# zhanwenchen/pbe

Hardware: AMD Instinct MI355X
Metric: 512x512 images/sec @50 PLMS steps scale=5 (higher is better)
Workload: dtype fp16; 1 GPU; BASELINE configs[1]: batch=4/GPU, 512x512, 50 PLMS steps (51 U-Net calls at batch 8), scale=5, fp16 activations + fp32 accumulate, name-seeded random-init U-Net + VAE + CLIP ViT-L/14 weights; the context-independent prefix of each guidance pair (first ResBlock + first self-attention) is evaluated once; per_gpu_batch=4, global_batch=4, plms_steps=50, parallelism=batch-sharded x1, no per-step collective

## Files before the change

### pbe_amd/csrc/attention.hip

```cpp
#include "common.h"
#include "../../include/pbe_hip.h"

struct AttnP {
    const h16* Q; const h16* K; const h16* VT; h16* O;
    int B, H, Nq, Nk, D;
    long q_bs, q_rs, k_bs, k_rs, vt_bs, vt_rs, o_bs, o_rs;
    float scale_log2e;
    int q_pre;
    int nqb;
#ifdef PBE_ATTN_STAMPS
    unsigned long long* stamps;
#endif
};

#define PBE_GLDS16(gsrc, ldst)                                                                     \
    __builtin_amdgcn_global_load_lds((const __attribute__((address_space(1))) void*)(gsrc),         \
                                     (__attribute__((address_space(3))) void*)(ldst), 16, 0, 0)

template <int DP>
struct AttnTile {
    static constexpr int KT = 64;
    static constexpr int DV = (DP + 31) / 32 * 32;
    static constexpr int DC = DP / 8;
    static constexpr int KR = DC | 1;
// ... 13 lines not shown
#endif

template <int DP, int QW, int KH, bool MPAD = false>
__global__ void __launch_bounds__(256, (QW == 2 && DP <= 48) ? 2 : 1) attn_kernel(const AttnP p) {
    using T = AttnTile<DP>;
    constexpr int KT = T::KT, DV = T::DV, KR = T::KR, VR = T::VR, KSTR = T::KSTR, VSTR = T::VSTR;
    constexpr int KSLOTS = T::KSLOTS, SLOTS = T::SLOTS, NPW = T::NPW, BUF = T::BUF;
    constexpr int K_BYTES = KSLOTS * 16;
    constexpr int NDS = DP / 16;
    constexpr int NDT = DV / 32;
    constexpr int BQ = 128 * QW;
    constexpr int NSLOT = 2 * KH;
    extern __shared__ __attribute__((aligned(16))) unsigned char smem[];

    const int tid = threadIdx.x, lane = tid & 63, wave = tid >> 6;
    const int l31 = lane & 31, h5 = lane >> 5;
    int bh, qblk;
    {
        const int nq = p.nqb, nbh = p.B * p.H, lin = blockIdx.x;
        if ((nbh & 7) == 0) { const int xcd = lin & 7, j = lin >> 3; qblk = j % nq; bh = (j / nq) * 8 + xcd; }
        else { qblk = lin % nq; bh = lin / nq; }
    }
    const int b = bh / p.H, h = bh - b * p.H;
    const int q0 = qblk * BQ + wave * 32 * QW + l31;
    const int D = p.D;
    const h16x8 zero8 = {0, 0, 0, 0, 0, 0, 0, 0};
    const h16x8 one8 = {1, 1, 1, 1, 1, 1, 1, 1};
    constexpr bool ONES = DV > DP;

    const h16* Qb = p.Q + (long)b * p.q_bs + (long)h * D;
    const h16* Kb = p.K + (long)b * p.k_bs + (long)h * D;
    const h16* Vb = p.VT + (long)b * p.vt_bs + (long)h * D * p.vt_rs;

    for (int i = tid; i < NSLOT * BUF / 16; i += 256) *reinterpret_cast<h16x8*>(smem + i * 16) = zero8;
    __syncthreads();
    if (ONES && tid < 8 * NSLOT)
        *reinterpret_cast<h16x8*>(smem + (tid >> 3) * BUF + K_BYTES + (DV - 1) * VSTR + (tid & 7) * 16) = one8;
    if constexpr (MPAD) {
        const h16x8 kpad = {(h16)64.f, 0, 0, 0, 0, 0, 0, 0};
        for (int i = tid; i < NSLOT * KT; i += 256)
            *reinterpret_cast<h16x8*>(smem + (i / KT) * BUF + (i % KT) * KSTR + (T::DC - 1) * 16) = kpad;
    }

    const h16* src[NPW];
    int inc[NPW];
#pragma unroll
    for (int j = 0; j < NPW; ++j) {
        const int slot = (j * 4 + wave) * 64 + lane;
        src[j] = nullptr; inc[j] = 0;
        if (slot < KSLOTS) {
            const int row = slot / KR, c = slot - row * KR;
            if (c * 8 < D) { src[j] = Kb + (long)attn_key_of_row(row) * p.k_rs + c * 8; inc[j] = KT * (int)p.k_rs; }
        } else if (slot < SLOTS) {
            const int sv = slot - KSLOTS, row = sv / VR, c = sv - row * VR;
            if (c < KT / 8 && row < D) { src[j] = Vb + (long)row * p.vt_rs + c * 8; inc[j] = KT; }
        }
    }
    const int nt = (p.Nk + KT - 1) / KT;
    const int rem = p.Nk - (nt - 1) * KT;
    auto issue_tile = [&](int t, int buf) {
        unsigned char* dst = smem + buf * BUF + wave * 1024;
        if (t + 1 < nt || rem == KT) {
#pragma unroll
            for (int j = 0; j < NPW; ++j) {
                if (src[j]) PBE_GLDS16(src[j], dst + j * 4096);
                src[j] += inc[j];
            }
        } else {
            const int kv0 = t * KT;
#pragma unroll
            for (int j = 0; j < NPW; ++j) {
                const int slot = (j * 4 + wave) * 64 + lane;
                const h16* s = nullptr;
                if (slot < KSLOTS) {
                    const int row = slot / KR, c = slot - row * KR;
                    const int key = min(kv0 + attn_key_of_row(row), p.Nk - 1);
                    if (c * 8 < D) s = Kb + (long)key * p.k_rs + c * 8;
                } else if (slot < SLOTS) {
                    const int sv = slot - KSLOTS, row = sv / VR, c = sv - row * VR;
                    if (c < KT / 8 && row < D && kv0 + c * 8 < p.Nk) s = Vb + (long)row * p.vt_rs + kv0 + c * 8;
                }
                if (s) PBE_GLDS16(s, dst + j * 4096);
            }
        }
    };
    auto fix_tail = [&](int buf) {
        unsigned char* sv = smem + buf * BUF + K_BYTES;
        for (int i = tid; i < DV * KT; i += 256) {
            const int row = i >> 6, col = i & 63;
            if (col >= rem) *reinterpret_cast<h16*>(sv + row * VSTR + col * 2) = (h16)0.f;
        }
    };

    h16x8 qf[QW][NDS];
#pragma unroll
    for (int i = 0; i < QW; ++i)
#pragma unroll
        for (int ds = 0; ds < NDS; ++ds) {
            const int d0 = ds * 16 + 8 * h5;
            const bool ok = (q0 + 32 * i) < p.Nq && d0 < D;
            const h16* qsrc = ok ? Qb + (long)(q0 + 32 * i) * p.q_rs + d0 : p.Q;
            h16x8 v = *reinterpret_cast<const h16x8*>(qsrc);
            v = ok ? v : zero8;
            if constexpr (MPAD) {
                if (!p.q_pre) {
#pragma unroll
                    for (int e = 0; e < 8; ++e) v[e] = (h16)((float)v[e] * p.scale_log2e);
                }
            }
            qf[i][ds] = v;
        }

    f32x16 o[QW][NDT];
    float m_run[QW], l_run[QW];
#pragma unroll
    for (int i = 0; i < QW; ++i) {
        m_run[i] = MPAD ? 0.f : -INFINITY; l_run[i] = 0.f;
#pragma unroll
        for (int dt = 0; dt < NDT; ++dt)
#pragma unroll
            for (int r = 0; r < 16; ++r) o[i][dt][r] = 0.f;
    }

    __syncthreads();
#pragma unroll
    for (int j = 0; j < KH; ++j)
        if (j < nt) issue_tile(j, j);
    __syncthreads();
    if (nt <= KH && rem < KT) { fix_tail(nt - 1); __syncthreads(); }

    constexpr bool PREF = DP <= 64, PREFV = DP <= 80;
    f32x16 sc[2];
    h16x8 pf[4];
    h16x8 kf[PREF ? 2 : 1][PREF ? NDS : 1];
    h16x8 vf[PREFV ? NDT : 1][4];
    auto load_k = [&](const unsigned char* sk) {
        if constexpr (PREF) {
#pragma unroll
            for (int ds = 0; ds < NDS; ++ds) {
                kf[0][ds] = *reinterpret_cast<const h16x8*>(sk + l31 * KSTR + (ds * 2 + h5) * 16);
                kf[1][ds] = *reinterpret_cast<const h16x8*>(sk + (32 + l31) * KSTR + (ds * 2 + h5) * 16);
            }
        }
    };
    auto load_v = [&](const unsigned char* sv) {
        if constexpr (PREFV) {
#pragma unroll
            for (int dt = 0; dt < NDT; ++dt)
#pragma unroll
                for (int ks = 0; ks < 4; ++ks)
                    vf[dt][ks] = *reinterpret_cast<const h16x8*>(sv + (dt * 32 + l31) * VSTR + h5 * 16 + ks * 32);
        }
    };
    auto qk = [&](int i, const unsigned char* sk) {
        f32x16& s0 = sc[0];
        f32x16& s1 = sc[1];
#pragma unroll
        for (int r = 0; r < 16; ++r) { s0[r] = 0.f; s1[r] = 0.f; }
        if constexpr (PREF) {
#pragma unroll
// ... 264 lines not shown
```

### pbe_amd/csrc/igemm.hip

```cpp
#include "igemm_kernel.h"

#ifdef PBE_STAMPS
unsigned long long* g_pbe_stamps = nullptr;
extern "C" int pbe_debug_set_stamps(void* buf) { g_pbe_stamps = (unsigned long long*)buf; return PBE_OK; }
#endif
int g_pbe_force_cfg = -1;
int g_pbe_allow_splitk = 1;
int g_pbe_pingpong = 1;
int g_pbe_mfast = 1;

extern "C" int pbe_tune(int32_t key, int32_t value) {
    if (key == 1) { g_pbe_force_cfg = (value >= 0 && (value & 255) < kNCfg) ? value : -1; return PBE_OK; }
    if (key == 2) { g_pbe_allow_splitk = value ? 1 : 0; return PBE_OK; }
    if (key == 3) { extern int g_pbe_attn_qw; g_pbe_attn_qw = value; return PBE_OK; }
    if (key == 4) { g_pbe_pingpong = value ? 1 : 0; return PBE_OK; }
    if (key == 5) { g_pbe_mfast = value ? 1 : 0; return PBE_OK; }
    if (key == 8) { extern int g_pbe_attn_pad_lds; g_pbe_attn_pad_lds = value > 0 ? value : 0; return PBE_OK; }
    if (key == 7) { extern int g_pbe_gn_rows; g_pbe_gn_rows = value >= 1 ? value : 16; return PBE_OK; }
    if (key == 10) { extern int g_pbe_gn_apply2_rows; g_pbe_gn_apply2_rows = value >= 0 ? value : 8; return PBE_OK; }
    if (key == 9) { extern int g_pbe_gn_apply_rows; g_pbe_gn_apply_rows = value >= 1 ? value : 4; return PBE_OK; }
    if (key == 6) { extern int g_pbe_attn_mpad; g_pbe_attn_mpad = value ? 1 : 0; return PBE_OK; }
    return pbe_set_error(PBE_EINVAL, "pbe_tune: unknown key %d", key);
}

static int fill_gemm(const pbe_gemm_desc* d, IGemmP& p, const char* who) {
    PBE_REQUIRE(d && d->A && d->W && d->C, "%s: null operand", who);
    PBE_REQUIRE(d->M > 0 && d->N > 0 && d->K > 0 && d->batch >= 1 && d->batch <= 65535, "%s: bad dims M=%d N=%d K=%d batch=%d", who, d->M, d->N, d->K, d->batch);
    PBE_REQUIRE(d->K % 8 == 0, "%s: K=%d must be a multiple of 8", who, d->K);
    PBE_REQUIRE(d->lda % 8 == 0 && d->ldw % 8 == 0 && al16(d->A) && al16(d->W), "%s: A/W must be 16-byte aligned with ld %% 8 == 0", who);
    PBE_REQUIRE(d->strideA % 8 == 0 && d->strideW % 8 == 0, "%s: batch strides of A/W must be multiples of 8", who);
    const int K1 = d->A2 ? d->K1 : d->K;
    if (d->A2) {
        PBE_REQUIRE(K1 > 0 && K1 < d->K && K1 % 32 == 0 && d->lda2 % 8 == 0 && al16(d->A2) && d->batch == 1,
                    "%s: split-K source needs K1 %% 32 == 0 (K1=%d), aligned A2, batch 1", who, K1);
    }
    PBE_REQUIRE(d->lda >= (d->A2 ? K1 : d->K) && d->ldw >= d->K, "%s: leading dims too small", who);
    PBE_REQUIRE(!d->rowvec || d->group_rows > 0, "%s: rowvec needs group_rows > 0", who);
    const bool geglu = d->act == PBE_ACT_GEGLU;
    const int Nout = geglu ? d->N / 2 : d->N;
    PBE_REQUIRE(!geglu || (d->N % 16 == 0 && !d->resid && !d->rowvec && !d->bias_per_row), "%s: GEGLU epilogue needs N %% 16 == 0 and no resid/rowvec", who);
    memset(&p, 0, sizeof(p));
    p.A = (const h16*)d->A; p.A2 = (const h16*)d->A2; p.W = (const h16*)d->W; p.C = (h16*)d->C;
    p.bias = d->bias; p.rowvec = (const h16*)d->rowvec; p.resid = (const h16*)d->resid;
    p.M = d->M; p.N = d->N; p.K = d->K; p.K1 = K1;
    p.lda = d->lda; p.lda2 = d->lda2; p.ldw = d->ldw; p.ldc = d->ldc; p.ldr = d->ldr;
    p.ldv = d->ldv; p.group_rows = d->group_rows > 0 ? d->group_rows : 1;
    p.sA = d->strideA; p.sW = d->strideW; p.sC = d->strideC; p.sR = d->strideR;
    p.alpha = d->alpha; p.act = d->act; p.bias_row = d->bias_per_row;
    PBE_REQUIRE(d->ldc >= (d->VT ? d->vt_col0 : Nout), "%s: ldc too small", who);
    p.vec = (Nout % 8 == 0) && (d->ldc % 8 == 0) && al16(d->C) && (d->strideC % 8 == 0) &&
            (!d->resid || ((d->ldr % 8 == 0) && al16(d->resid) && (d->strideR % 8 == 0)));
    p.ws = (float*)d->workspace;
    p.alpha_cols = d->alpha_cols;
// ... 229 lines not shown
```

### pbe_amd/csrc/igemm_kernel.h

```cpp
#pragma once
#include <type_traits>
#include <utility>
#include "common.h"
#include "../../include/pbe_hip.h"

struct IGemmP {
    const h16* A; const h16* A2; const h16* W; h16* C;
    const float* bias; const h16* rowvec; const h16* resid;
    int M, N, K, K1;
    long lda, lda2, ldw, ldc, ldr;
    int ldv, group_rows;
    long sA, sW, sC, sR;
    float alpha; int act; int bias_row; int vec;
    int H, Wd, C1, C2, Ho, Wo, cstride, pad, ups, cb;
    int phase;
    int th;
    const float* sa; const float* sw; long ssa, ssw;
    int splits; float* ws;
    int alpha_cols;
    const float* ln_stat;
    int ln_parts; long ln_ld;
    const float* ln_c1; float ln_eps; double ln_inv_k;
    long rstat_ld;
    float* rstat;
// ... 199 lines not shown
    constexpr int PA = BM / 8, PW = BN / 8;
    constexpr int LA = PA / NW, LW = (PW + NW - 1) / NW, LPT = LA + LW;
    constexpr int CLD = BN + 8;
    constexpr int RING = MODE == 2 ? 2 * HPA * 128 + S * W_BYTES : S * STAGE;
    static_assert(S >= 2 && S <= 4 && PA % NW == 0 && BM % 16 == 0 && BN % 16 == 0, "A pieces must divide over the waves (weight pieces may be padded)");
    static_assert(MODE != 2 || (HPA % 8 == 0 && HPA >= BM), "halo image must hold the tile");
    static_assert(EXF == 0 || (MODE == 0 && !F8), "extended epilogue: dense fp16 tiles only");
    static_assert(!EXM || (MODE == 0 && !EXS && (F8 || EXF == (EX_LN | EX_VT))), "MX-fp8 copy-out: the fp8 tiles and the q|k|v^T form");
    extern __shared__ __attribute__((aligned(16))) unsigned char smem[];

    const int tid = threadIdx.x, lane = tid & 63;
    const int wave = __builtin_amdgcn_readfirstlane(tid >> 6);
    const int wm = wave % NWM, wn = wave / NWM;
    PBE_ACC_DECL;
#if PBE_PRIO_MODE == 2
    if (NW == 8 && __builtin_amdgcn_readfirstlane(wave) >= 4) __builtin_amdgcn_s_setprio(1);
#endif
    PBE_STAMP(0);
    PBE_STAMP(7);
    int tile;
    {
        const int nwg = gridDim.x, id = blockIdx.x, q = nwg >> 3, r = nwg & 7, xcd = id & 7;
        tile = (xcd < r ? xcd * (q + 1) : r * (q + 1) + (xcd - r) * q) + (id >> 3);
    }
    const int tiles_m = gridDim.x / tiles_n;
    const int tn_i = p.m_fast ? tile / tiles_m : tile % tiles_n, tm_i = p.m_fast ? tile - tn_i * tiles_m : tile / tiles_n;
    const int m0 = tm_i * BM, n0 = tn_i * BN;
    const long bz = blockIdx.y;

    const int lrow = lane >> 3;
    const int gch = (lane & 7) ^ lrow;
    const h16* zsrc = reinterpret_cast<const h16*>(g_pbe_zero16);

    const h16* a_cur[LA];
    const h16* a_alt[LA];
#pragma unroll
    for (int i = 0; i < LA; ++i) {
        const int m = min(m0 + (wave * LA + i) * 8 + lrow, p.M - 1);
        a_cur[i] = p.A + bz * p.sA + (long)m * p.lda + gch * 8;
        a_alt[i] = p.A2 ? p.A2 + (long)m * p.lda2 + gch * 8 - p.K1 : a_cur[i];
    }
    int* tab = reinterpret_cast<int*>(smem + RING);
    float* svec = reinterpret_cast<float*>(smem + (RING > WM * CLD * 2 ? RING : WM * CLD * 2) + (MODE == 1 ? 9 * BM * 4 : 0));
    const int sv_ns = (p.rowvec && p.group_rows < BM) ? BM / p.group_rows : 1;
    if (MODE == 1) {
        const int hw = p.Ho * p.Wo, Hv = p.H << p.ups, Wv = p.Wd << p.ups;
        const int py = p.phase ? (int)(blockIdx.y >> 1) : 0, px = p.phase ? (int)(blockIdx.y & 1) : 0;
        for (int row = tid; row < BM; row += NT) {
            const int m = m0 + row;
            const bool rok = m < p.M;
            const int b = m / hw, rem = m - b * hw;
            const int oy = rem / p.Wo, ox = rem - oy * p.Wo;
            const int iy0 = oy * p.cstride - p.pad, ix0 = ox * p.cstride - p.pad;
            if (p.phase) {
#pragma unroll
                for (int tp = 0; tp < 4; ++tp) {
                    const int iy = oy - 1 + py + (tp >> 1), ix = ox - 1 + px + (tp & 1);
                    const bool ok = rok && (unsigned)iy < (unsigned)p.H && (unsigned)ix < (unsigned)p.Wd;
                    tab[tp * BM + row] = ok ? (b * p.H + iy) * p.Wd + ix : -1;
                }
                continue;
            }
#pragma unroll
            for (int tp = 0; tp < 9; ++tp) {
                const int iy = iy0 + tp / 3, ix = ix0 + tp % 3;
                const bool ok = rok && (unsigned)iy < (unsigned)Hv && (unsigned)ix < (unsigned)Wv;
                tab[tp * BM + row] = ok ? (b * p.H + (iy >> p.ups)) * p.Wd + (ix >> p.ups) : -1;
            }
        }
        __syncthreads();
    }
    const h16* w_row[LW];
#pragma unroll
    for (int i = 0; i < LW; ++i) {
        const int n = min(n0 + min(wave + NW * i, PW - 1) * 8 + lrow, p.N - 1);
        w_row[i] = p.W + bz * p.sW + (long)n * p.ldw + gch * 8;
    }
    const int nk_all = (p.K + 63) >> 6;
    int kt0 = 0, nk = nk_all;
    if (p.splits > 1) {
        const int per = (nk_all + p.splits - 1) / p.splits;
        kt0 = blockIdx.z * per;
        nk = min(nk_all, kt0 + per);
    }
    const int KB = MODE == 1 ? p.cb >> 6 : 1;
    const int ntap = (MODE == 1 && p.phase) ? 4 : 9;
    int tap = 0, c0 = 0, kj = 0;
    if (MODE == 1 && kt0 > 0) {
        const int per_blk = ntap * KB, cblk = kt0 / per_blk, r = kt0 - cblk * per_blk;
        tap = r / KB; kj = r - tap * KB; c0 = cblk * p.cb + kj * 64;
    }
    const h16* a_src[LA];
    int a_inc[LA];
    bool fresh = true;
#pragma unroll
    for (int i = 0; i < LA; ++i) { a_src[i] = zsrc; a_inc[i] = 0; }
    const bool ktail = (p.K & 63) != 0, straddle = p.A2 && (p.K1 & 63);
    const int kt_sw = p.A2 ? p.K1 >> 6 : 0x7fffffff;
    if (MODE == 0 && kt0 > kt_sw) {
#pragma unroll
        for (int i = 0; i < LA; ++i) a_cur[i] = a_alt[i];
    }

    auto issue = [&](int kt, int slot) {
        unsigned char* sa = smem + slot * STAGE;
        unsigned char* sw = sa + A_BYTES;
        const long k = (long)kt * 64;
        const bool slow = (ktail && kt == nk_all - 1) || (straddle && kt == kt_sw);
        const int kl = kt * 64 + gch * 8;
        if (MODE == 0) {
            if (kt == kt_sw && !straddle) {
#pragma unroll
                for (int i = 0; i < LA; ++i) a_cur[i] = a_alt[i];
            }
            if (!slow) {
#pragma unroll
                for (int i = 0; i < LA; ++i) PBE_GLDS16(a_cur[i] + k, sa + (wave * LA + i) * 1024);
            } else {
#pragma unroll
                for (int i = 0; i < LA; ++i) {
                    const h16* src = (kl < p.K1 ? a_cur[i] : a_alt[i]) + k;
                    PBE_GLDS16(kl < p.K ? src : zsrc, sa + (wave * LA + i) * 1024);
                }
                if (straddle && kt == kt_sw) {
#pragma unroll
                    for (int i = 0; i < LA; ++i) a_cur[i] = a_alt[i];
                }
            }
        } else {
            if (kj == 0 || fresh) {
                fresh = false;
                const bool first = c0 < p.C1;
                const h16* base = first ? p.A + c0 + gch * 8 : p.A2 + (c0 - p.C1) + gch * 8;
                const long cs = first ? p.C1 : p.C2;
#pragma unroll
                for (int i = 0; i < LA; ++i) {
                    const int pix = tab[tap * BM + (wave * LA + i) * 8 + lrow];
                    a_src[i] = pix >= 0 ? base + (long)pix * cs : zsrc;
                    a_inc[i] = pix >= 0 ? 64 : 0;
                }
            }
#pragma unroll
            for (int i = 0; i < LA; ++i) {
                PBE_GLDS16(a_src[i], sa + (wave * LA + i) * 1024);
                a_src[i] += a_inc[i];
            }
            c0 += 64;
            if (++kj == KB) {
                kj = 0;
                if (++tap == ntap) tap = 0; else c0 -= p.cb;
            }
        }
        if (!slow) {
#pragma unroll
            for (int i = 0; i < LW; ++i) PBE_GLDS16(w_row[i] + k, sw + min(wave + NW * i, PW - 1) * 1024);
        } else {
#pragma unroll
            for (int i = 0; i < LW; ++i) PBE_GLDS16(kl < p.K ? w_row[i] + k : zsrc, sw + min(wave + NW * i, PW - 1) * 1024);
        }
    };

    f32x4 acc[TN][TM];
#pragma unroll
    for (int i = 0; i < TN; ++i)
#pragma unroll
        for (int j = 0; j < TM; ++j) acc[i][j] = (f32x4){0.f, 0.f, 0.f, 0.f};

    const int fr = lane & 15, fq = lane >> 4;
    const int rsw = (fq ^ (fr & 7)) << 4;
    const int a_rd = (wm * WM + fr) * 128, w_rd = (wn * WN + fr) * 128;

    float* sca = svec + 4 * BN;
    float* scw = sca + BM;
    float* lnc = scw + BM;
    auto stage_svec = [&]() {
        if constexpr (F8) {
            for (int idx = tid; idx < BM + BN; idx += NT) {
                float v = 1.f;
                if (idx < BM) { if (p.sa && m0 + idx < p.M) v = p.sa[bz * p.ssa + m0 + idx]; sca[idx] = v; }
                else { const int c = idx - BM; if (p.sw && n0 + c < p.N) v = p.sw[bz * p.ssw + n0 + c]; scw[c] = v; }
            }
        }
        if constexpr (EXL) {
            if (p.ln_stat) {
                for (int idx = tid; idx < BM + BN; idx += NT) {
                    if (idx < BM) {
                        const int m = min(m0 + idx, p.M - 1);
                        float a = 0.f, q = 0.f;
                        for (int z = 0; z < p.ln_parts; ++z) {
                            const float2 t = *reinterpret_cast<const float2*>(p.ln_stat + 2 * ((long)z * p.ln_ld + m));
                            a += t.x; q += t.y;
                        }
                        const double mean = (double)a * p.ln_inv_k;
// ... 280 lines not shown
                            fa[ks][j] = *reinterpret_cast<const h16x8*>(ab + arow[j] * 128 + (((ks * 4 + fq) ^ (arow[j] & 7)) << 4));
#pragma unroll
                        for (int i = 0; i < TN; ++i) fw[ks][i] = *reinterpret_cast<const h16x8*>(sw + w_rd + (rsw ^ (ks * 64)) + i * 16 * 128);
                    }
                    __builtin_amdgcn_sched_barrier(0);
                    if (kt + D < nk2) issue_w(kt + D, slot_wr);
                    if (tap == 0 && next_a) issue_a(blk + 1, (blk + 1 - blk0) & 1);
                    __builtin_amdgcn_sched_barrier(0);
                    PBE_SETPRIO(1);
#pragma unroll
                    for (int i = 0; i < TN; ++i)
#pragma unroll
                        for (int j = 0; j < TM; ++j)
                            acc[i][j] = __builtin_amdgcn_mfma_f32_16x16x32_f16(fw[0][i], fa[0][j], acc[i][j], 0, 0, 0);
                    if constexpr (!BOTH) {
#pragma unroll
                        for (int j = 0; j < TM; ++j)
                            fa[0][j] = *reinterpret_cast<const h16x8*>(ab + arow[j] * 128 + (((4 + fq) ^ (arow[j] & 7)) << 4));
#pragma unroll
                        for (int i = 0; i < TN; ++i) fw[0][i] = *reinterpret_cast<const h16x8*>(sw + w_rd + (rsw ^ 64) + i * 16 * 128);
                    }
#pragma unroll
                    for (int i = 0; i < TN; ++i)
#pragma unroll
                        for (int j = 0; j < TM; ++j)
                            acc[i][j] = __builtin_amdgcn_mfma_f32_16x16x32_f16(fw[BOTH ? 1 : 0][i], fa[BOTH ? 1 : 0][j], acc[i][j], 0, 0, 0);
                    PBE_SETPRIO(0);
                    slot_rd = slot_rd + 1 == S ? 0 : slot_rd + 1;
                    slot_wr = slot_wr + 1 == S ? 0 : slot_wr + 1;
                }
            }
        }
    } else {
    PBE_STAMP(1);
#pragma unroll
    for (int t = 0; t < D; ++t)
        if (kt0 + t < nk) issue(kt0 + t, t);
    PBE_STAMP(2);
    stage_svec();
    int slot_rd = 0, slot_wr = D % S;
    for (int kt = kt0; kt < nk; ++kt) {
#ifdef PBE_STAMPS
        if (kt == kt0 + 1) PBE_STAMP(3);
#endif
        const int rem = min(nk - 1 - kt, D - 1);
        PBE_ACC_T0();
        if (D >= 3 && rem >= 2) wait_vmcnt<2 * LPT>();
        else if (D >= 2 && rem >= 1) wait_vmcnt<LPT>();
        else wait_vmcnt<0>();
        PBE_ACC(acc_w_);
        asm volatile("s_waitcnt lgkmcnt(0)" ::: "memory");
        PBE_ACC_T0();
        __builtin_amdgcn_s_barrier();
        PBE_ACC(acc_b2_);
        PBE_ACC_T0();
        const unsigned char* sa = smem + slot_rd * STAGE;
        const unsigned char* sw = sa + A_BYTES;
        h16x8 fa[BOTH ? 2 : 1][TM], fw[BOTH ? 2 : 1][TN];
#pragma unroll
        for (int ks = 0; ks < (BOTH ? 2 : 1); ++ks) {
#pragma unroll
            for (int j = 0; j < TM; ++j) fa[ks][j] = *reinterpret_cast<const h16x8*>(sa + a_rd + (rsw ^ (ks * 64)) + j * 16 * 128);
#pragma unroll
            for (int i = 0; i < TN; ++i) fw[ks][i] = *reinterpret_cast<const h16x8*>(sw + w_rd + (rsw ^ (ks * 64)) + i * 16 * 128);
        }
        __builtin_amdgcn_sched_barrier(0);
        if (kt + D < nk) issue(kt + D, slot_wr);
        __builtin_amdgcn_sched_barrier(0);
        PBE_ACC(acc_r_);
// ... 667 lines not shown
```

### pbe_amd/csrc/norm.hip

```cpp
#include "common.h"
#include "../../include/pbe_hip.h"

#define GN_MAX_C 4096
#define GN_MAX_CHUNKS 256

__device__ __forceinline__ const h16* gn_src(const h16* X, const h16* X2, int C1, int C2, long row, int v) {
    const int c = v * 8;
    return (c < C1) ? X + row * C1 + c : X2 + row * C2 + (c - C1);
}

__global__ void __launch_bounds__(256) gn_stats_kernel(const h16* X, const h16* X2, float* part, int HW, int C1, int C2,
                                                        int groups, int rows_per_block, int TX, int TY) {
    __shared__ float s_sum[GN_MAX_C], s_sq[GN_MAX_C];
    __shared__ float s_pa[256 * 8], s_pq[256 * 8];
    const int C = C1 + C2, C8 = C >> 3, cg = C / groups;
    const int tid = threadIdx.x, tx = tid % TX, ty = tid / TX;
    const int b = blockIdx.y, chunk = blockIdx.x;
    const int r0 = chunk * rows_per_block;
    const int r1 = min(HW, r0 + rows_per_block);
    if (ty < TY) {
        for (int v = tx; v < C8; v += TX) {
            float a[8], q[8];
#pragma unroll
            for (int e = 0; e < 8; ++e) { a[e] = 0.f; q[e] = 0.f; }
// ... 9 lines not shown
            }
            for (; r < r1; r += TY) {
                const h16x8 x = *reinterpret_cast<const h16x8*>(gn_src(X, X2, C1, C2, (long)b * HW + r, v));
#pragma unroll
                for (int e = 0; e < 8; ++e) { const float f = (float)x[e]; a[e] += f; q[e] += f * f; }
            }
            if (TY == 1) {
#pragma unroll
                for (int e = 0; e < 8; ++e) { s_sum[v * 8 + e] = a[e]; s_sq[v * 8 + e] = q[e]; }
            } else {
#pragma unroll
                for (int e = 0; e < 8; ++e) { s_pa[tid * 8 + e] = a[e]; s_pq[tid * 8 + e] = q[e]; }
            }
        }
    }
    __syncthreads();
    if (TY > 1) {
        for (int c = tid; c < C; c += 256) {
            const int v = c >> 3, e = c & 7;
            float a = 0.f, q = 0.f;
            for (int y = 0; y < TY; ++y) { a += s_pa[(y * TX + v) * 8 + e]; q += s_pq[(y * TX + v) * 8 + e]; }
            s_sum[c] = a; s_sq[c] = q;
        }
        __syncthreads();
    }
    if (tid < groups) {
        float a = 0.f, q = 0.f;
        for (int c = tid * cg; c < (tid + 1) * cg; ++c) { a += s_sum[c]; q += s_sq[c]; }
        float* dst = part + (((long)b * gridDim.x + chunk) * groups + tid) * 2;
        dst[0] = a; dst[1] = q;
    }
}

__global__ void __launch_bounds__(256) gn_apply_kernel(const h16* X, const h16* X2, const float* part, const float* gamma,
                                                        const float* beta, h16* Y, int HW, int C1, int C2, int groups,
                                                        int nchunks, int rows_per_block, int TX, int TY, float eps, int silu) {
    __shared__ float s_mean[64], s_rstd[64];
    __shared__ double s_a[256], s_q[256];
    const int C = C1 + C2, C8 = C >> 3, cg = C / groups;
    const int tid = threadIdx.x, tx = tid % TX, ty = tid / TX;
    const int b = blockIdx.y;
    {
        const int slices = 256 / groups;
        const int g = tid % groups, sl = tid / groups;
        double a = 0.0, q = 0.0;
        if (sl < slices)
            for (int c = sl; c < nchunks; c += slices) {
                const float* src = part + (((long)b * nchunks + c) * groups + g) * 2;
                a += (double)src[0]; q += (double)src[1];
            }
        s_a[tid] = a; s_q[tid] = q;
        __syncthreads();
        if (tid < groups) {
            double ta = 0.0, tq = 0.0;
            for (int s = 0; s < slices; ++s) { ta += s_a[s * groups + tid]; tq += s_q[s * groups + tid]; }
            const double n = (double)HW * cg;
            const double mean = ta / n;
            double var = tq / n - mean * mean;
            if (var < 0.0) var = 0.0;
            s_mean[tid] = (float)mean;
            s_rstd[tid] = (float)(1.0 / sqrt(var + (double)eps));
        }
        __syncthreads();
    }
    const int r0 = blockIdx.x * rows_per_block;
    const int r1 = min(HW, r0 + rows_per_block);
    if (ty >= TY) return;
    for (int v = tx; v < C8; v += TX) {
        float sc[8], sh[8];
#pragma unroll
        for (int e = 0; e < 8; ++e) {
            const int c = v * 8 + e, g = c / cg;
            const float a = s_rstd[g] * gamma[c];
            sc[e] = a; sh[e] = beta[c] - s_mean[g] * a;
        }
        int r = r0 + ty;
        for (; r + 3 * TY < r1; r += 4 * TY) {
            h16x8 x[4];
#pragma unroll
            for (int u = 0; u < 4; ++u) x[u] = *reinterpret_cast<const h16x8*>(gn_src(X, X2, C1, C2, (long)b * HW + r + u * TY, v));
#pragma unroll
            for (int u = 0; u < 4; ++u) {
                h16x8 y;
#pragma unroll
                for (int e = 0; e < 8; ++e) {
                    float f = (float)x[u][e] * sc[e] + sh[e];
                    if (silu) f = silu_f(f);
                    y[e] = (h16)f;
                }
                *reinterpret_cast<h16x8*>(Y + ((long)b * HW + r + u * TY) * C + v * 8) = y;
            }
        }
        for (; r < r1; r += TY) {
            const long row = (long)b * HW + r;
            const h16x8 x = *reinterpret_cast<const h16x8*>(gn_src(X, X2, C1, C2, row, v));
            h16x8 y;
#pragma unroll
            for (int e = 0; e < 8; ++e) {
                float f = (float)x[e] * sc[e] + sh[e];
                if (silu) f = silu_f(f);
                y[e] = (h16)f;
            }
            *reinterpret_cast<h16x8*>(Y + row * C + v * 8) = y;
        }
    }
}

#define GN_SMALL_ROWS 12
__global__ void __launch_bounds__(256) gn_small_kernel(const h16* X, const h16* X2, const float* gamma, const float* beta, h16* Y,
                                                        int HW, int C1, int C2, int groups, float eps, int silu) {
    __shared__ float s_a[4], s_q[4];
    const int C = C1 + C2, cg = C / groups, TX = cg >> 3, TY = 256 / TX;
    const int tid = threadIdx.x, lane = tid & 63, wave = tid >> 6;
    const int tx = tid % TX, ty = tid / TX;
    const int g = blockIdx.x, b = blockIdx.y;
    const int v = (g * cg >> 3) + tx;
    const bool act = ty < TY;
    h16x8 x[GN_SMALL_ROWS];
    float a = 0.f, q = 0.f;
#pragma unroll
    for (int u = 0; u < GN_SMALL_ROWS; ++u) {
        const int r = ty + u * TY;
        if (act && r < HW) {
            x[u] = *reinterpret_cast<const h16x8*>(gn_src(X, X2, C1, C2, (long)b * HW + r, v));
#pragma unroll
            for (int e = 0; e < 8; ++e) { const float f = (float)x[u][e]; a += f; q += f * f; }
        }
    }
    a = wave_sum(a); q = wave_sum(q);
    if (lane == 0) { s_a[wave] = a; s_q[wave] = q; }
    __syncthreads();
    const double n = (double)HW * cg;
    const double mean = ((double)s_a[0] + s_a[1] + s_a[2] + s_a[3]) / n;
    double var = ((double)s_q[0] + s_q[1] + s_q[2] + s_q[3]) / n - mean * mean;
    if (var < 0.0) var = 0.0;
    const float mu = (float)mean, rstd = (float)(1.0 / sqrt(var + (double)eps));
    if (!act) return;
    float sc[8], sh[8];
#pragma unroll
    for (int e = 0; e < 8; ++e) {
        const int c = v * 8 + e;
        sc[e] = rstd * gamma[c];
        sh[e] = beta[c] - mu * sc[e];
    }
#pragma unroll
    for (int u = 0; u < GN_SMALL_ROWS; ++u) {
        const int r = ty + u * TY;
        if (r < HW) {
            h16x8 y;
#pragma unroll
            for (int e = 0; e < 8; ++e) {
                float f = (float)x[u][e] * sc[e] + sh[e];
                if (silu) f = silu_f(f);
                y[e] = (h16)f;
            }
            *reinterpret_cast<h16x8*>(Y + ((long)b * HW + r) * C + v * 8) = y;
        }
    }
}

int g_pbe_gn_rows = 16;
int g_pbe_gn_apply2_rows = 8;
int g_pbe_gn_apply_rows = 4;
static void gn_geometry(int HW, int C, int* nchunks, int* rpb, int* TX, int* TY, int rows_per_thread = 0) {
    const int C8 = C / 8;
    *TX = C8 < 256 ? C8 : 256;
    *TY = 256 / *TX;
    int rows = *TY * (rows_per_thread > 0 ? rows_per_thread : g_pbe_gn_rows);
    if (rows < 32) rows = 32;
    int n = (HW + rows - 1) / rows;
    if (n > GN_MAX_CHUNKS) { n = GN_MAX_CHUNKS; rows = (HW + n - 1) / n; n = (HW + rows - 1) / rows; }
    *nchunks = n; *rpb = rows;
}

extern "C" size_t pbe_groupnorm_workspace_bytes(int32_t B, int32_t HW) {
    (void)HW;
    return (size_t)B * GN_MAX_CHUNKS * 64 * 2 * sizeof(float);
}

extern "C" int pbe_groupnorm_f16(const void* X, const void* X2, const float* gamma, const float* beta, void* Y, int32_t B,
                                 int32_t HW, int32_t C1, int32_t C2, int32_t groups, float eps, int32_t silu, void* workspace,
                                 size_t workspace_bytes, pbe_stream_t stream) {
    const int C = C1 + C2;
    PBE_REQUIRE(X && gamma && beta && Y && workspace, "pbe_groupnorm_f16: null operand");
    PBE_REQUIRE(B > 0 && HW > 0 && C1 > 0 && C2 >= 0, "pbe_groupnorm_f16: bad dims");
    PBE_REQUIRE((C2 == 0) == (X2 == nullptr), "pbe_groupnorm_f16: X2 / C2 mismatch");
    PBE_REQUIRE(C1 % 8 == 0 && C2 % 8 == 0 && C <= GN_MAX_C, "pbe_groupnorm_f16: C1=%d C2=%d must be multiples of 8, total <= %d", C1, C2, GN_MAX_C);
    PBE_REQUIRE(groups > 0 && groups <= 64 && C % groups == 0, "pbe_groupnorm_f16: groups=%d must divide C=%d (<= 64)", groups, C);
    PBE_REQUIRE(B <= 65535, "pbe_groupnorm_f16: batch too large");
    PBE_REQUIRE(workspace_bytes >= pbe_groupnorm_workspace_bytes(B, HW), "pbe_groupnorm_f16: workspace too small");
    hipStream_t s = (hipStream_t)stream;
    const int cg = C / groups;
    if (cg % 8 == 0 && cg / 8 <= 64 && HW <= GN_SMALL_ROWS * (256 / (cg / 8))) {
        pbe_prof_begin(PBE_K_GNORM, s);
        hipLaunchKernelGGL(gn_small_kernel, dim3(groups, B), dim3(256), 0, s, (const h16*)X, (const h16*)X2, gamma, beta, (h16*)Y, HW, C1, C2,
                           groups, eps, silu);
        pbe_prof_end(PBE_K_GNORM, s, 4.0 * B * (double)HW * C);
        PBE_LAUNCH_CHECK("pbe_groupnorm_f16");
        return PBE_OK;
    }
    int nchunks, rpb, TX, TY;
    gn_geometry(HW, C, &nchunks, &rpb, &TX, &TY);
    pbe_prof_begin(PBE_K_GNORM, s);
    hipLaunchKernelGGL(gn_stats_kernel, dim3(nchunks, B), dim3(256), 0, s, (const h16*)X, (const h16*)X2, (float*)workspace, HW, C1, C2,
                       groups, rpb, TX, TY);
    {
        int ac = nchunks, arpb = rpb, aTX = TX, aTY = TY;
        if (g_pbe_gn_apply2_rows > 0) gn_geometry(HW, C, &ac, &arpb, &aTX, &aTY, g_pbe_gn_apply2_rows);
        hipLaunchKernelGGL(gn_apply_kernel, dim3(ac, B), dim3(256), 0, s, (const h16*)X, (const h16*)X2, (const float*)workspace, gamma,
                           beta, (h16*)Y, HW, C1, C2, groups, nchunks, arpb, aTX, aTY, eps, silu);
    }
    pbe_prof_end(PBE_K_GNORM, s, 6.0 * B * (double)HW * C);
    PBE_LAUNCH_CHECK("pbe_groupnorm_f16");
    return PBE_OK;
}

extern "C" int pbe_groupnorm_apply_f16(const void* X, const float* partials, int32_t blocks, const float* gamma, const float* beta, void* Y,
                                       int32_t B, int32_t HW, int32_t C, int32_t groups, float eps, int32_t silu, pbe_stream_t stream) {
    PBE_REQUIRE(X && partials && gamma && beta && Y, "pbe_groupnorm_apply_f16: null operand");
    PBE_REQUIRE(B > 0 && B <= 65535 && HW > 0 && C > 0 && C % 8 == 0 && C <= GN_MAX_C && blocks > 0, "pbe_groupnorm_apply_f16: bad dims");
    PBE_REQUIRE(groups > 0 && groups <= 64 && C % groups == 0, "pbe_groupnorm_apply_f16: groups=%d must divide C=%d (<= 64)", groups, C);
    hipStream_t s = (hipStream_t)stream;
    int nchunks, rpb, TX, TY;
    gn_geometry(HW, C, &nchunks, &rpb, &TX, &TY, g_pbe_gn_apply_rows);
    pbe_prof_begin(PBE_K_GNORM, s);
    hipLaunchKernelGGL(gn_apply_kernel, dim3(nchunks, B), dim3(256), 0, s, (const h16*)X, (const h16*)nullptr, partials, gamma, beta, (h16*)Y, HW, C, 0,
                       groups, blocks, rpb, TX, TY, eps, silu);
    pbe_prof_end(PBE_K_GNORM, s, 4.0 * B * (double)HW * C);
    PBE_LAUNCH_CHECK("pbe_groupnorm_apply_f16");
    return PBE_OK;
}

template <int VPL>
__global__ void __launch_bounds__(256) layernorm_kernel(const h16* X, const float* gamma, const float* beta, h16* Y, long rows, int C,
                                                         long ldx, long ldy, float eps) {
    const int lane = threadIdx.x & 63;
    const long row = (long)blockIdx.x * 4 + (threadIdx.x >> 6);
    if (row >= rows) return;
    const int C8 = C >> 3;
    h16x8 x[VPL];
    float sum = 0.f;
#pragma unroll
    for (int i = 0; i < VPL; ++i) {
        const int v = lane + 64 * i;
        if (v < C8) {
            x[i] = *reinterpret_cast<const h16x8*>(X + row * ldx + v * 8);
#pragma unroll
            for (int e = 0; e < 8; ++e) sum += (float)x[i][e];
        }
    }
    const float mean = wave_sum(sum) / (float)C;
    float sq = 0.f;
#pragma unroll
    for (int i = 0; i < VPL; ++i) {
        const int v = lane + 64 * i;
        if (v < C8) {
#pragma unroll
// ... 207 lines not shown
```

Baseline: 7.923 images/sec.

## Hoist global loads ahead of LDS init in attention, igemm, and groupnorm kernels

In attention, Q fragments and the first K/V tile loads are issued before the shared-memory padding initialisation, which now writes only the pad regions. In igemm, the first weight tile load is issued before the A-address table build. Groupnorm apply and small kernels prefetch X rows and load gamma/beta as vectors before the statistics reduction, with a 4-way unrolled partial-sum read. The goal is to hide global-load latency behind setup work. Default apply rows and minimum rows change, launch bounds are added, and gamma/beta must now be 16-byte aligned, which adds register pressure and a new alignment requirement.

```diff
diff --git a/pbe_amd/csrc/attention.hip b/pbe_amd/csrc/attention.hip
--- a/pbe_amd/csrc/attention.hip
+++ b/pbe_amd/csrc/attention.hip
@@ -69,15 +69,16 @@
     const h16* Kb = p.K + (long)b * p.k_bs + (long)h * D;
     const h16* Vb = p.VT + (long)b * p.vt_bs + (long)h * D * p.vt_rs;
 
-    for (int i = tid; i < NSLOT * BUF / 16; i += 256) *reinterpret_cast<h16x8*>(smem + i * 16) = zero8;
-    __syncthreads();
-    if (ONES && tid < 8 * NSLOT)
-        *reinterpret_cast<h16x8*>(smem + (tid >> 3) * BUF + K_BYTES + (DV - 1) * VSTR + (tid & 7) * 16) = one8;
-    if constexpr (MPAD) {
-        const h16x8 kpad = {(h16)64.f, 0, 0, 0, 0, 0, 0, 0};
-        for (int i = tid; i < NSLOT * KT; i += 256)
-            *reinterpret_cast<h16x8*>(smem + (i / KT) * BUF + (i % KT) * KSTR + (T::DC - 1) * 16) = kpad;
-    }
+    h16x8 qf[QW][NDS];
+#pragma unroll
+    for (int i = 0; i < QW; ++i)
+#pragma unroll
+        for (int ds = 0; ds < NDS; ++ds) {
+            const int d0 = ds * 16 + 8 * h5;
+            const bool ok = (q0 + 32 * i) < p.Nq && d0 < D;
+            qf[i][ds] = *reinterpret_cast<const h16x8*>(ok ? Qb + (long)(q0 + 32 * i) * p.q_rs + d0 : p.Q);
+        }
+    __builtin_amdgcn_sched_barrier(0);
 
     const h16* src[NPW];
     int inc[NPW];
@@ -129,16 +130,41 @@
         }
     };
 
-    h16x8 qf[QW][NDS];
+#pragma unroll
+    for (int j = 0; j < KH; ++j)
+        if (j < nt) issue_tile(j, j);
+    __builtin_amdgcn_sched_barrier(0);
+
+    {
+        const int D8 = D >> 3, kz = KR - D8, nkz = KT * kz, nvz = (DV - D) * VR, per = nkz + nvz + D;
+        const h16x8 kpad = {(h16)64.f, 0, 0, 0, 0, 0, 0, 0};
+        for (int i = tid; i < NSLOT * per; i += 256) {
+            const int img = i / per;
+            int r = i - img * per, off;
+            h16x8 val = zero8;
+            if (r < nkz) {
+                const int row = r / kz, c = D8 + (r - row * kz);
+                off = row * KSTR + c * 16;
+                if (MPAD && c == T::DC - 1) val = kpad;
+            } else {
+                r -= nkz;
+                int row, c;
+                if (r < nvz) { const int rr = r / VR; row = D + rr; c = r - rr * VR; }
+                else { row = r - nvz; c = VR - 1; }
+                off = K_BYTES + row * VSTR + c * 16;
+                if (ONES && row == DV - 1 && c < KT / 8) val = one8;
+            }
+            *reinterpret_cast<h16x8*>(smem + img * BUF + off) = val;
+        }
+    }
+
 #pragma unroll
     for (int i = 0; i < QW; ++i)
 #pragma unroll
         for (int ds = 0; ds < NDS; ++ds) {
             const int d0 = ds * 16 + 8 * h5;
             const bool ok = (q0 + 32 * i) < p.Nq && d0 < D;
-            const h16* qsrc = ok ? Qb + (long)(q0 + 32 * i) * p.q_rs + d0 : p.Q;
-            h16x8 v = *reinterpret_cast<const h16x8*>(qsrc);
-            v = ok ? v : zero8;
+            h16x8 v = ok ? qf[i][ds] : zero8;
             if constexpr (MPAD) {
                 if (!p.q_pre) {
 #pragma unroll
@@ -159,10 +185,6 @@
             for (int r = 0; r < 16; ++r) o[i][dt][r] = 0.f;
     }
 
-    __syncthreads();
-#pragma unroll
-    for (int j = 0; j < KH; ++j)
-        if (j < nt) issue_tile(j, j);
     __syncthreads();
     if (nt <= KH && rem < KT) { fix_tail(nt - 1); __syncthreads(); }
 
diff --git a/pbe_amd/csrc/igemm.hip b/pbe_amd/csrc/igemm.hip
--- a/pbe_amd/csrc/igemm.hip
+++ b/pbe_amd/csrc/igemm.hip
@@ -18,7 +18,7 @@
     if (key == 8) { extern int g_pbe_attn_pad_lds; g_pbe_attn_pad_lds = value > 0 ? value : 0; return PBE_OK; }
     if (key == 7) { extern int g_pbe_gn_rows; g_pbe_gn_rows = value >= 1 ? value : 16; return PBE_OK; }
     if (key == 10) { extern int g_pbe_gn_apply2_rows; g_pbe_gn_apply2_rows = value >= 0 ? value : 8; return PBE_OK; }
-    if (key == 9) { extern int g_pbe_gn_apply_rows; g_pbe_gn_apply_rows = value >= 1 ? value : 4; return PBE_OK; }
+    if (key == 9) { extern int g_pbe_gn_apply_rows; g_pbe_gn_apply_rows = value >= 1 ? value : 8; return PBE_OK; }
     if (key == 6) { extern int g_pbe_attn_mpad; g_pbe_attn_mpad = value ? 1 : 0; return PBE_OK; }
     return pbe_set_error(PBE_EINVAL, "pbe_tune: unknown key %d", key);
 }
diff --git a/pbe_amd/csrc/igemm_kernel.h b/pbe_amd/csrc/igemm_kernel.h
--- a/pbe_amd/csrc/igemm_kernel.h
+++ b/pbe_amd/csrc/igemm_kernel.h
@@ -255,6 +255,40 @@
     const int gch = (lane & 7) ^ lrow;
     const h16* zsrc = reinterpret_cast<const h16*>(g_pbe_zero16);
 
+    const h16* w_row[LW];
+#pragma unroll
+    for (int i = 0; i < LW; ++i) {
+        const int n = min(n0 + min(wave + NW * i, PW - 1) * 8 + lrow, p.N - 1);
+        w_row[i] = p.W + bz * p.sW + (long)n * p.ldw + gch * 8;
+    }
+    const int nk_all = (p.K + 63) >> 6;
+    int kt0 = 0, nk = nk_all;
+    if (p.splits > 1) {
+        const int per = (nk_all + p.splits - 1) / p.splits;
+        kt0 = blockIdx.z * per;
+        nk = min(nk_all, kt0 + per);
+    }
+    const bool ktail = (p.K & 63) != 0, straddle = p.A2 && (p.K1 & 63);
+    const int kt_sw = p.A2 ? p.K1 >> 6 : 0x7fffffff;
+    auto issue_wt = [&](int kt, int slot) {
+        unsigned char* sw = smem + slot * STAGE + A_BYTES;
+        const long k = (long)kt * 64;
+        const bool slow = (ktail && kt == nk_all - 1) || (straddle && kt == kt_sw);
+        const int kl = kt * 64 + gch * 8;
+        if (!slow) {
+#pragma unroll
+            for (int i = 0; i < LW; ++i) PBE_GLDS16(w_row[i] + k, sw + min(wave + NW * i, PW - 1) * 1024);
+        } else {
+#pragma unroll
+            for (int i = 0; i < LW; ++i) PBE_GLDS16(kl < p.K ? w_row[i] + k : zsrc, sw + min(wave + NW * i, PW - 1) * 1024);
+        }
+    };
+    if constexpr (MODE != 2) {
+        PBE_STAMP(1);
+        if (kt0 < nk) issue_wt(kt0, 0);
+        __builtin_amdgcn_sched_barrier(0);
+    }
+
     const h16* a_cur[LA];
     const h16* a_alt[LA];
 #pragma unroll
@@ -291,20 +325,8 @@
                 tab[tp * BM + row] = ok ? (b * p.H + (iy >> p.ups)) * p.Wd + (ix >> p.ups) : -1;
             }
         }
-        __syncthreads();
-    }
-    const h16* w_row[LW];
-#pragma unroll
-    for (int i = 0; i < LW; ++i) {
-        const int n = min(n0 + min(wave + NW * i, PW - 1) * 8 + lrow, p.N - 1);
-        w_row[i] = p.W + bz * p.sW + (long)n * p.ldw + gch * 8;
-    }
-    const int nk_all = (p.K + 63) >> 6;
-    int kt0 = 0, nk = nk_all;
-    if (p.splits > 1) {
-        const int per = (nk_all + p.splits - 1) / p.splits;
-        kt0 = blockIdx.z * per;
-        nk = min(nk_all, kt0 + per);
+        asm volatile("s_waitcnt lgkmcnt(0)" ::: "memory");
+        __builtin_amdgcn_s_barrier();
     }
     const int KB = MODE == 1 ? p.cb >> 6 : 1;
     const int ntap = (MODE == 1 && p.phase) ? 4 : 9;
@@ -318,16 +340,13 @@
     bool fresh = true;
 #pragma unroll
     for (int i = 0; i < LA; ++i) { a_src[i] = zsrc; a_inc[i] = 0; }
-    const bool ktail = (p.K & 63) != 0, straddle = p.A2 && (p.K1 & 63);
-    const int kt_sw = p.A2 ? p.K1 >> 6 : 0x7fffffff;
     if (MODE == 0 && kt0 > kt_sw) {
 #pragma unroll
         for (int i = 0; i < LA; ++i) a_cur[i] = a_alt[i];
     }
 
-    auto issue = [&](int kt, int slot) {
+    auto issue_at = [&](int kt, int slot) {
         unsigned char* sa = smem + slot * STAGE;
-        unsigned char* sw = sa + A_BYTES;
         const long k = (long)kt * 64;
         const bool slow = (ktail && kt == nk_all - 1) || (straddle && kt == kt_sw);
         const int kl = kt * 64 + gch * 8;
@@ -374,14 +393,8 @@
                 if (++tap == ntap) tap = 0; else c0 -= p.cb;
             }
         }
-        if (!slow) {
-#pragma unroll
-            for (int i = 0; i < LW; ++i) PBE_GLDS16(w_row[i] + k, sw + min(wave + NW * i, PW - 1) * 1024);
-        } else {
-#pragma unroll
-            for (int i = 0; i < LW; ++i) PBE_GLDS16(kl < p.K ? w_row[i] + k : zsrc, sw + min(wave + NW * i, PW - 1) * 1024);
-        }
     };
+    auto issue = [&](int kt, int slot) { issue_at(kt, slot); issue_wt(kt, slot); };
 
     f32x4 acc[TN][TM];
 #pragma unroll
@@ -728,9 +741,9 @@
             }
         }
     } else {
-    PBE_STAMP(1);
-#pragma unroll
-    for (int t = 0; t < D; ++t)
+    if (kt0 < nk) issue_at(kt0, 0);
+#pragma unroll
+    for (int t = 1; t < D; ++t)
         if (kt0 + t < nk) issue(kt0 + t, t);
     PBE_STAMP(2);
     stage_svec();
diff --git a/pbe_amd/csrc/norm.hip b/pbe_amd/csrc/norm.hip
--- a/pbe_amd/csrc/norm.hip
+++ b/pbe_amd/csrc/norm.hip
@@ -65,7 +65,7 @@
     }
 }
 
-__global__ void __launch_bounds__(256) gn_apply_kernel(const h16* X, const h16* X2, const float* part, const float* gamma,
+__global__ void __launch_bounds__(256, 4) gn_apply_kernel(const h16* X, const h16* X2, const float* part, const float* gamma,
                                                         const float* beta, h16* Y, int HW, int C1, int C2, int groups,
                                                         int nchunks, int rows_per_block, int TX, int TY, float eps, int silu) {
     __shared__ float s_mean[64], s_rstd[64];
@@ -73,14 +73,36 @@
     const int C = C1 + C2, C8 = C >> 3, cg = C / groups;
     const int tid = threadIdx.x, tx = tid % TX, ty = tid / TX;
     const int b = blockIdx.y;
+    const int r0 = blockIdx.x * rows_per_block;
+    const int r1 = min(HW, r0 + rows_per_block);
+    const bool act = ty < TY && tx < C8;
+    h16x8 x[4];
+    f32x4 g0, g1, b0, b1;
+    if (act) {
+#pragma unroll
+        for (int u = 0; u < 4; ++u) {
+            const int r = r0 + ty + u * TY;
+            if (r < r1) x[u] = *reinterpret_cast<const h16x8*>(gn_src(X, X2, C1, C2, (long)b * HW + r, tx));
+        }
+        g0 = *reinterpret_cast<const f32x4*>(gamma + tx * 8); g1 = *reinterpret_cast<const f32x4*>(gamma + tx * 8 + 4);
+        b0 = *reinterpret_cast<const f32x4*>(beta + tx * 8); b1 = *reinterpret_cast<const f32x4*>(beta + tx * 8 + 4);
+    }
     {
         const int slices = 256 / groups;
         const int g = tid % groups, sl = tid / groups;
         double a = 0.0, q = 0.0;
         if (sl < slices)
-            for (int c = sl; c < nchunks; c += slices) {
-                const float* src = part + (((long)b * nchunks + c) * groups + g) * 2;
-                a += (double)src[0]; q += (double)src[1];
+            for (int c = sl; c < nchunks; c += 4 * slices) {
+                float pa[4], pq[4];
+#pragma unroll
+                for (int u = 0; u < 4; ++u) {
+                    const int cu = c + u * slices;
+                    const float* src = part + (((long)b * nchunks + (cu < nchunks ? cu : c)) * groups + g) * 2;
+                    pa[u] = src[0]; pq[u] = src[1];
+                }
+#pragma unroll
+                for (int u = 0; u < 4; ++u)
+                    if (c + u * slices < nchunks) { a += (double)pa[u]; q += (double)pq[u]; }
             }
         s_a[tid] = a; s_q[tid] = q;
         __syncthreads();
@@ -96,45 +118,44 @@
         }
         __syncthreads();
     }
-    const int r0 = blockIdx.x * rows_per_block;
-    const int r1 = min(HW, r0 + rows_per_block);
-    if (ty >= TY) return;
+    if (!act) return;
+    const float rcg = 1.0f / (float)cg;
     for (int v = tx; v < C8; v += TX) {
+        if (v != tx) {
+            g0 = *reinterpret_cast<const f32x4*>(gamma + v * 8); g1 = *reinterpret_cast<const f32x4*>(gamma + v * 8 + 4);
+            b0 = *reinterpret_cast<const f32x4*>(beta + v * 8); b1 = *reinterpret_cast<const f32x4*>(beta + v * 8 + 4);
+        }
         float sc[8], sh[8];
+        int g = (int)((float)(v * 8) * rcg);
+        int rem = v * 8 - g * cg;
+        if (rem < 0) { --g; rem += cg; } else if (rem >= cg) { ++g; rem -= cg; }
 #pragma unroll
         for (int e = 0; e < 8; ++e) {
-            const int c = v * 8 + e, g = c / cg;
-            const float a = s_rstd[g] * gamma[c];
-            sc[e] = a; sh[e] = beta[c] - s_mean[g] * a;
-        }
-        int r = r0 + ty;
-        for (; r + 3 * TY < r1; r += 4 * TY) {
-            h16x8 x[4];
-#pragma unroll
-            for (int u = 0; u < 4; ++u) x[u] = *reinterpret_cast<const h16x8*>(gn_src(X, X2, C1, C2, (long)b * HW + r + u * TY, v));
+            const float a = s_rstd[g] * (e < 4 ? g0[e & 3] : g1[e & 3]);
+            sc[e] = a; sh[e] = (e < 4 ? b0[e & 3] : b1[e & 3]) - s_mean[g] * a;
+            if (++rem == cg) { rem = 0; ++g; }
+        }
+        bool loaded = v == tx;
+        for (int r = r0 + ty; r < r1; r += 4 * TY) {
+            if (!loaded) {
+#pragma unroll
+                for (int u = 0; u < 4; ++u)
+                    if (r + u * TY < r1) x[u] = *reinterpret_cast<const h16x8*>(gn_src(X, X2, C1, C2, (long)b * HW + r + u * TY, v));
+            }
+            loaded = false;
 #pragma unroll
             for (int u = 0; u < 4; ++u) {
-                h16x8 y;
-#pragma unroll
-                for (int e = 0; e < 8; ++e) {
-                    float f = (float)x[u][e] * sc[e] + sh[e];
-                    if (silu) f = silu_f(f);
-                    y[e] = (h16)f;
+                if (r + u * TY < r1) {
+                    h16x8 y;
+#pragma unroll
+                    for (int e = 0; e < 8; ++e) {
+                        float f = (float)x[u][e] * sc[e] + sh[e];
+                        if (silu) f = silu_f(f);
+                        y[e] = (h16)f;
+                    }
+                    *reinterpret_cast<h16x8*>(Y + ((long)b * HW + r + u * TY) * C + v * 8) = y;
                 }
-                *reinterpret_cast<h16x8*>(Y + ((long)b * HW + r + u * TY) * C + v * 8) = y;
-            }
-        }
-        for (; r < r1; r += TY) {
-            const long row = (long)b * HW + r;
-            const h16x8 x = *reinterpret_cast<const h16x8*>(gn_src(X, X2, C1, C2, row, v));
-            h16x8 y;
-#pragma unroll
-            for (int e = 0; e < 8; ++e) {
-                float f = (float)x[e] * sc[e] + sh[e];
-                if (silu) f = silu_f(f);
-                y[e] = (h16)f;
-            }
-            *reinterpret_cast<h16x8*>(Y + row * C + v * 8) = y;
+            }
         }
     }
 }
@@ -150,12 +171,21 @@
     const int v = (g * cg >> 3) + tx;
     const bool act = ty < TY;
     h16x8 x[GN_SMALL_ROWS];
+#pragma unroll
+    for (int u = 0; u < GN_SMALL_ROWS; ++u) {
+        const int r = ty + u * TY;
+        if (act && r < HW) x[u] = *reinterpret_cast<const h16x8*>(gn_src(X, X2, C1, C2, (long)b * HW + r, v));
+    }
+    f32x4 g0, g1, b0, b1;
+    if (act) {
+        g0 = *reinterpret_cast<const f32x4*>(gamma + v * 8); g1 = *reinterpret_cast<const f32x4*>(gamma + v * 8 + 4);
+        b0 = *reinterpret_cast<const f32x4*>(beta + v * 8); b1 = *reinterpret_cast<const f32x4*>(beta + v * 8 + 4);
+    }
     float a = 0.f, q = 0.f;
 #pragma unroll
     for (int u = 0; u < GN_SMALL_ROWS; ++u) {
         const int r = ty + u * TY;
         if (act && r < HW) {
-            x[u] = *reinterpret_cast<const h16x8*>(gn_src(X, X2, C1, C2, (long)b * HW + r, v));
 #pragma unroll
             for (int e = 0; e < 8; ++e) { const float f = (float)x[u][e]; a += f; q += f * f; }
         }
@@ -172,9 +202,8 @@
     float sc[8], sh[8];
 #pragma unroll
     for (int e = 0; e < 8; ++e) {
-        const int c = v * 8 + e;
-        sc[e] = rstd * gamma[c];
-        sh[e] = beta[c] - mu * sc[e];
+        sc[e] = rstd * (e < 4 ? g0[e & 3] : g1[e & 3]);
+        sh[e] = (e < 4 ? b0[e & 3] : b1[e & 3]) - mu * sc[e];
     }
 #pragma unroll
     for (int u = 0; u < GN_SMALL_ROWS; ++u) {
@@ -194,13 +223,13 @@
 
 int g_pbe_gn_rows = 16;
 int g_pbe_gn_apply2_rows = 8;
-int g_pbe_gn_apply_rows = 4;
-static void gn_geometry(int HW, int C, int* nchunks, int* rpb, int* TX, int* TY, int rows_per_thread = 0) {
+int g_pbe_gn_apply_rows = 8;
+static void gn_geometry(int HW, int C, int* nchunks, int* rpb, int* TX, int* TY, int rows_per_thread = 0, int min_rows = 32) {
     const int C8 = C / 8;
     *TX = C8 < 256 ? C8 : 256;
     *TY = 256 / *TX;
     int rows = *TY * (rows_per_thread > 0 ? rows_per_thread : g_pbe_gn_rows);
-    if (rows < 32) rows = 32;
+    if (rows < min_rows) rows = min_rows;
     int n = (HW + rows - 1) / rows;
     if (n > GN_MAX_CHUNKS) { n = GN_MAX_CHUNKS; rows = (HW + n - 1) / n; n = (HW + rows - 1) / rows; }
     *nchunks = n; *rpb = rows;
@@ -222,6 +251,7 @@
     PBE_REQUIRE(groups > 0 && groups <= 64 && C % groups == 0, "pbe_groupnorm_f16: groups=%d must divide C=%d (<= 64)", groups, C);
     PBE_REQUIRE(B <= 65535, "pbe_groupnorm_f16: batch too large");
     PBE_REQUIRE(workspace_bytes >= pbe_groupnorm_workspace_bytes(B, HW), "pbe_groupnorm_f16: workspace too small");
+    PBE_REQUIRE(((uintptr_t)gamma & 15) == 0 && ((uintptr_t)beta & 15) == 0, "pbe_groupnorm_f16: gamma / beta must be 16-byte aligned");
     hipStream_t s = (hipStream_t)stream;
     const int cg = C / groups;
     if (cg % 8 == 0 && cg / 8 <= 64 && HW <= GN_SMALL_ROWS * (256 / (cg / 8))) {
@@ -239,7 +269,7 @@
                        groups, rpb, TX, TY);
     {
         int ac = nchunks, arpb = rpb, aTX = TX, aTY = TY;
-        if (g_pbe_gn_apply2_rows > 0) gn_geometry(HW, C, &ac, &arpb, &aTX, &aTY, g_pbe_gn_apply2_rows);
+        if (g_pbe_gn_apply2_rows > 0) gn_geometry(HW, C, &ac, &arpb, &aTX, &aTY, g_pbe_gn_apply2_rows, 1);
         hipLaunchKernelGGL(gn_apply_kernel, dim3(ac, B), dim3(256), 0, s, (const h16*)X, (const h16*)X2, (const float*)workspace, gamma,
                            beta, (h16*)Y, HW, C1, C2, groups, nchunks, arpb, aTX, aTY, eps, silu);
     }
@@ -253,9 +283,10 @@
     PBE_REQUIRE(X && partials && gamma && beta && Y, "pbe_groupnorm_apply_f16: null operand");
     PBE_REQUIRE(B > 0 && B <= 65535 && HW > 0 && C > 0 && C % 8 == 0 && C <= GN_MAX_C && blocks > 0, "pbe_groupnorm_apply_f16: bad dims");
     PBE_REQUIRE(groups > 0 && groups <= 64 && C % groups == 0, "pbe_groupnorm_apply_f16: groups=%d must divide C=%d (<= 64)", groups, C);
+    PBE_REQUIRE(((uintptr_t)gamma & 15) == 0 && ((uintptr_t)beta & 15) == 0, "pbe_groupnorm_apply_f16: gamma / beta must be 16-byte aligned");
     hipStream_t s = (hipStream_t)stream;
     int nchunks, rpb, TX, TY;
-    gn_geometry(HW, C, &nchunks, &rpb, &TX, &TY, g_pbe_gn_apply_rows);
+    gn_geometry(HW, C, &nchunks, &rpb, &TX, &TY, g_pbe_gn_apply_rows, 1);
     pbe_prof_begin(PBE_K_GNORM, s);
     hipLaunchKernelGGL(gn_apply_kernel, dim3(nchunks, B), dim3(256), 0, s, (const h16*)X, (const h16*)nullptr, partials, gamma, beta, (h16*)Y, HW, C, 0,
                        groups, blocks, rpb, TX, TY, eps, silu);
```

New measurement: 8.006 images/sec, median of 6. 1.01x the previous value.
